# KamikaziZen/admm-quantization

Measured on AMD Instinct MI355X. Metric: ADMM iters/sec, resnet18 all conv layers 4-bit r=2.0; rel-Frob err vs CPU ref, higher is better.
Workload: dtype f32

## Files before the change

### admm-quantization_amd/admmq/_lib.py

```python
from __future__ import annotations

import ctypes
import os
from typing import Sequence

import torch

_HERE = os.path.dirname(os.path.abspath(__file__))
LIB_PATH = os.environ.get("ADMMQ_LIB") or os.path.join(_HERE, "libadmmq.so")

SCHEMES = {
    "tensor_mseminmax_symmetric": 0,
    "tensor_minmax": 1,
    "tensor_symmetric": 2,
    "tensor_affine": 3,
}
CHANNEL_SCHEMES = {"channel_symmetric": 4, "channel_affine": 5}


class AdmmProblem(ctypes.Structure):
    _fields_ = [("F", ctypes.c_void_p), ("G", ctypes.c_void_p), ("H0", ctypes.c_void_p),
                ("H_out", ctypes.c_void_p), ("U", ctypes.c_void_p), ("HT_out", ctypes.c_void_p),
                ("X_out", ctypes.c_void_p), ("I", ctypes.c_int32), ("R", ctypes.c_int32)]

# ... 41 lines not shown
def use_ops() -> bool:
    return not os.environ.get("ADMMQ_LIB")


def ops():
    global _ops
    if _ops is None:
        if not os.path.exists(OPS_PATH):
            raise ImportError(f"admmq: {OPS_PATH} is missing - build it with `make -C admm-quantization_amd/csrc`")
        load()
        torch.ops.load_library(OPS_PATH)
        _ops = torch.ops.admmq
    return _ops


def load() -> ctypes.CDLL:
    global _lib
    if _lib is not None:
        return _lib
    if not os.path.exists(LIB_PATH):
        raise ImportError(f"admmq: {LIB_PATH} is missing - build it with `python -c 'import __graft_entry__ as g; g.build()'` "
                          "or `make -C admm-quantization_amd/csrc`; there is no CPU fallback")
    lib = ctypes.CDLL(LIB_PATH)
    P, S, I32, I64, F32 = ctypes.c_void_p, ctypes.c_size_t, ctypes.c_int32, ctypes.c_int64, ctypes.c_float
    sig = {
        "admmq_admm_workspace_size": (S, [P, I32, I32]),
        "admmq_admm_prepare": (I32, [P, I32, I32, P, S, P]),
        "admmq_admm_run": (I32, [P, I32, I32, F32, I32, I32, I32, P, S, P, P]),
        "admmq_admm_iteration_batched": (I32, [P, I32, I32, F32, I32, I32, I32, P, S, P, P]),
        "admmq_admm_default_options": (I32, [P]),
        "admmq_admm_workspace_size_ex": (S, [P, I32, I32, P]),
        "admmq_admm_prepare_ex": (I32, [P, I32, I32, P, P, S, P]),
        "admmq_admm_run_ex": (I32, [P, I32, I32, F32, I32, I32, I32, P, P, S, P, P]),
        "admmq_debug_set_fin_wait_polls": (I32, [ctypes.c_uint32]),
        "admmq_debug_set_f32_persistent": (I32, [I32, I32]),
        "admmq_debug_set_gemm_ks": (I32, [I32]),
        "admmq_debug_set_gemm_stage": (I32, [I32]),
        "admmq_debug_set_ksplit": (I32, [I32]),
        "admmq_debug_set_ksplit_form": (I32, [I32]),
        "admmq_debug_set_ksplit_balance": (I32, [I32, I32]),
        "admmq_debug_ksplit_balance_count": (ctypes.c_int64, [ctypes.c_void_p, I32]),
        "admmq_debug_ksplit_pieces": (I32, [I32, I32]),
        "admmq_debug_set_even_units": (I32, [I32]),
        "admmq_spd_solve64": (I32, [P, P, I64, I64, P, P, P]),
        "admmq_debug_epc_evals": (I32, [P, I32]),
        "admmq_debug_spd_trace": (I32, [P]),
        "admmq_debug_epc_trace": (I32, [P]),
        "admmq_epc_step64": (I32, [P, P, I64, I64, ctypes.c_double, ctypes.c_double, P, P, P, P, P]),
        "admmq_debug_hist_cu": (I32, [P, I32]),
        "admmq_debug_set_fin_capacity": (I32, [I32]),
        "admmq_debug_set_fin_nv3": (I32, [I32]),
        "admmq_debug_set_thin_loop": (I32, [I32]),
        "admmq_quantize_workspace_size": (S, [P, I32, I32]),
        "admmq_quantize_batched": (I32, [P, I32, I32, I32, I32, P, S, P]),
        "admmq_packed_bytes": (S, [I64, I32]),
        "admmq_quantize_packed_workspace_size": (S, [P, I32, I32]),
        "admmq_quantize_packed": (I32, [P, P, P, I32, I32, I32, I32, P, S, P]),
        "admmq_dequantize_packed": (I32, [P, P, P, P, I32, P]),
        "admmq_packed_gemm_workspace_size": (S, [I64, I64, I64, I32]),
        "admmq_packed_gemm": (I32, [P, P, I32, I64, I64, P, I32, I64, I32, P, P, P, S, P]),
        "admmq_packed_dwgemm_workspace_size": (S, [I64, I64, I64, I64, I32]),
        "admmq_packed_dwgemm": (I32, [P, P, I64, I64, P, I32, I64, I64, P, I32, I32, I32, I32, I32, I32, P, P, P, S, P]),
        "admmq_fixed_quantize": (I32, [P, P, I64, P, P]),
        "admmq_packed_gemm_act": (I32, [P, P, I32, I64, I64, P, I32, I64, I32, P, P, P, P, S, P]),
        "admmq_packed_dwgemm_act": (I32, [P, P, I64, I64, P, I32, I64, I64, P, I32, I32, I32, I32, I32, I32, P, P, P, P, P,
                                          S, P]),
        "admmq_act_encode": (I32, [P, P, I64, P, P, P]),
        "admmq_act_decode": (I32, [P, P, I64, P, P]),
        "admmq_packed_rowsums": (I32, [P, P, I32, I64, I64, P, P]),
        "admmq_packed_igemm_workspace_size": (S, [I64, I64, I64, I32]),
        "admmq_packed_igemm": (I32, [P, P, I32, I64, I64, P, P, P, I32, I64, I32, P, P, P, P, P, P, S, P]),
        "admmq_mse_sse_table": (I32, [P, I64, I64, I32, I32, P, P, S, P]),
        "admmq_quantize_channel_workspace_size": (S, [P, I32, I32]),
        "admmq_quantize_channel": (I32, [P, P, P, I32, I32, I32, I32, P, S, P]),
        "admmq_set_exhaustive_search": (I32, [I32]),
        "admmq_debug_set_sel_widen": (I32, [I32]),
        "admmq_debug_shared_stage2_count": (I64, [I32]),
        "admmq_debug_set_wide_min_tiles": (I32, [ctypes.c_int64]),
        "admmq_set_solve_mode": (I32, [I32]),
        "admmq_get_solve_mode": (I32, []),
        "admmq_debug_set_legacy_stage1": (I32, [I32]),
        "admmq_debug_set_launch_head": (I32, [I32]),
        "admmq_debug_get_launch_head_default": (I32, []),
        "admmq_debug_admm_plan_bytes": (S, [P, I32, I32, P]),
        "admmq_debug_admm_plan_digest": (I32, [P, I32, I32, I32, P, P]),
        "admmq_debug_admm_run_schedule": (I32, [P, I32, I32, I32, I32, I32, I32, I32, I32, I32, P]),
        "admmq_debug_check_thresholds": (I32, [ctypes.c_uint32, I32]),
        "admmq_debug_set_fused_finalize": (I32, [I32]),
        "admmq_debug_set_search_units_per_block": (I32, [I32]),
        "admmq_debug_check_cells": (I32, [I32, I32, ctypes.c_uint32, I32, P]),
        "admmq_profile_begin": (I32, [I32, I32]),
        "admmq_profile_end": (I32, [P, P]),
        "admmq_cp_workspace_size": (S, [P, I32, I32]),
        "admmq_cp_gram_mttkrp": (I32, [P, I32, I32, P, S, P]),
        "admmq_cp_rel_error": (I32, [P, I32, P, P, S, P]),
        "admmq_cp64_workspace_size": (S, [P, I32, I32]),
        "admmq_cp64_gram_mttkrp": (I32, [P, I32, I32, P, S, P]),
        "admmq_lowrank_workspace_size": (S, [I64]),
        "admmq_lowrank_reset": (I32, [P, S, P]),
        "admmq_lowrank_pre": (I32, [P, P, P, P, P, P, I64, F32, P, S, P]),
        "admmq_lowrank_post": (I32, [P, P, P, P, I64, F32, P, S, P]),
        "admmq_panel_workspace_size": (S, [I64, I64, I64]),
        "admmq_panel_xtq": (I32, [P, I64, I64, I64, P, I64, P, P, S, P]),
        "admmq_panel_xy": (I32, [P, I64, I64, I64, P, I64, P, P, S, P]),
        "admmq_panel_outer": (I32, [P, P, I64, I64, I64, P, I64, P]),
        "admmq_gram64_workspace_size": (S, [I64, I64, I64]),
        "admmq_gram64": (I32, [P, I64, P, I64, I64, I64, I64, P, P, S, P]),
        "admmq_epc_mu": (I32, [P, P, I64, ctypes.c_double, ctypes.c_double, P, P]),
        "admmq_cp_colnorm64": (I32, [P, I64, P, I64, I64, P, P, P]),
        "admmq_solve64_workspace_size": (S, [I64, I64]),
        "admmq_epc64_max_evals": (I32, []),
        "admmq_debug_s64_evals": (I32, [P, I32]),
        "admmq_spd_solve64_ws": (I32, [P, P, I64, I64, ctypes.c_double, P, P, P, S, P]),
        "admmq_epc_begin64": (I32, [P, P, I64, I64, ctypes.c_double, ctypes.c_double, P, P, P, S, P]),
        "admmq_epc_rounds64": (I32, [P, P, I64, I64, P, I32, P, P, S, P]),
        "admmq_epc_end64": (I32, [I64, I64, P, P, P, S, P]),
        "admmq_version": (I32, []),
        "admmq_last_error": (ctypes.c_char_p, []),
    }
    for name, (res, args) in sig.items():
        if os.environ.get("ADMMQ_LIB") and not hasattr(lib, name):
            continue
        fn = getattr(lib, name)
        fn.restype = res
        fn.argtypes = args
    _lib = lib
    return lib


def check(rc: int, what: str):
    if rc != 0:
        msg = load().admmq_last_error().decode(errors="replace")
        raise RuntimeError(f"admmq: {what} failed (status {rc}): {msg}")


def require_device(*tensors: torch.Tensor):
    for t in tensors:
        if not isinstance(t, torch.Tensor):
            raise TypeError(f"admmq: expected a torch.Tensor, got {type(t).__name__}")
        if t.device.type != "cuda":
            raise RuntimeError("admmq: tensors must live on a ROCm GPU (device 'cuda'); the MI355X path has "
                               "no CPU implementation")
        if t.dtype != torch.float32:
            raise TypeError(f"admmq: float32 tensors required, got {t.dtype}")


def stream_handle(device: torch.device) -> ctypes.c_void_p:
    return ctypes.c_void_p(torch.cuda.current_stream(device).cuda_stream)


def ptr(t) -> ctypes.c_void_p:
    return ctypes.c_void_p(0 if t is None else t.data_ptr())


def workspace(nbytes: int, device: torch.device) -> torch.Tensor:
    return torch.empty(max(int(nbytes), 256), dtype=torch.uint8, device=device)


def problems_array(items: Sequence[AdmmProblem]):
    arr = (AdmmProblem * len(items))(*items)
    return arr


def qtensor_array(items: Sequence[QTensor]):
    return (QTensor * len(items))(*items)


_PY_REPAIRS = [0]


def note_repair(n: int = 1):
    _PY_REPAIRS[0] += n


def fault_repairs(reset: bool = False) -> int:
    n = _PY_REPAIRS[0]
    if reset:
        _PY_REPAIRS[0] = 0
    if use_ops():
        n += int(ops().fault_repairs(bool(reset)))
    return n


class _switch:

    _setter = ""
    _restore = 0
    _checked = (False, False)

    def _encode(self) -> int:
        return 1 if self.enable else 0

    def _set(self, value: int, checked: bool):
        rc = getattr(load(), self._setter)(value)
        if checked:
            check(rc, type(self).__name__)

    def __enter__(self):
        self._set(self._encode(), self._checked[0])
        return self

    def __exit__(self, *exc):
        self._set(self._restore, self._checked[1])
        return False


class exhaustive_search(_switch):

    _setter = "admmq_set_exhaustive_search"

    def __init__(self, enable: bool = True):
        self.enable = enable


class sel_widen(_switch):

    _setter, _checked = "admmq_debug_set_sel_widen", (True, True)

    def __init__(self, mode: int = 1):
        if mode not in (1, 2):
            raise ValueError(mode)
        self.mode = mode

    def _encode(self):
        return self.mode


def shared_stage2_count(reset: bool = False) -> int:
    n = int(load().admmq_debug_shared_stage2_count(1 if reset else 0))
    if n < 0:
        raise RuntimeError("admmq: shared_stage2_count failed")
    return n


class solve_mode:

    MODES = SOLVE_MODES

    def __init__(self, mode: str):
        if mode not in self.MODES:
            raise ValueError(mode)
        self.mode = mode

    def __enter__(self):
        self.prev = load().admmq_get_solve_mode()
        check(load().admmq_set_solve_mode(self.MODES[self.mode]), "set_solve_mode")
        return self

    def __exit__(self, *exc):
        load().admmq_set_solve_mode(self.prev)
        return False


class fin_nv3(_switch):

    _setter, _restore = "admmq_debug_set_fin_nv3", 1

    def __init__(self, enable: bool):
        self.enable = enable


class fused_finalize(_switch):

    _setter, _restore = "admmq_debug_set_fused_finalize", 1

    def __init__(self, enable: bool):
        self.enable = enable


class fin_wait_polls(_switch):

    _setter, _checked = "admmq_debug_set_fin_wait_polls", (True, False)

    def __init__(self, polls: int):
        self.polls = polls

    def _encode(self):
        return int(self.polls)


class fin_capacity(_switch):

    _setter, _checked = "admmq_debug_set_fin_capacity", (True, False)

    def __init__(self, blocks: int):
        self.blocks = blocks

    def _encode(self):
        return int(self.blocks)


class thin_loop(_switch):

    _setter, _restore, _checked = "admmq_debug_set_thin_loop", 1, (True, False)

    def __init__(self, enable):
        self.enable = enable

    def _encode(self):
        return 2 if self.enable == "wide" else (1 if self.enable else 0)


class search_units_per_block(_switch):

    _setter, _checked = "admmq_debug_set_search_units_per_block", (True, False)

    def __init__(self, reps: int):
        self.reps = reps

    def _encode(self):
# ... 15 lines not shown
```

### admm-quantization_amd/csrc/admmq_internal.h

```cpp
#pragma once
#include <hip/hip_runtime.h>
#include <stdint.h>

struct admmq_qmeta;

#ifndef ADMMQ_TRACE
#define ADMMQ_TRACE 0
#endif
#define ADMMQ_NOW() (ADMMQ_TRACE ? __builtin_amdgcn_s_memrealtime() : 0ull)

namespace admmq {

enum QScheme { kMse = 0, kMinMax = 1, kSymmetric = 2, kAffine = 3 };
enum SolveMode { kSolveF32 = 0, kSolveSplit = 1 };

constexpr int kMaxSel = 64;
constexpr int kMaxStage1 = 1024;
constexpr int kMaxStage1Bits = 6;
constexpr int kHistRep = 8;
constexpr int kMaxMerged = 4096;
constexpr int kCells = 4096;
constexpr int kResRep = 8;
constexpr int kThinRows = 16;
constexpr long long kWideMinTiles = 4 * 768;
constexpr int kWideRows = 256;

struct MseView {
  const float* X;
  const float* U;
  int rows, cols, ld, qpr;
  int nq, nelem;
  unsigned* stat;
  unsigned long long* sse;
  unsigned long long* h1;
  unsigned long long* h2;
  double* s2;
  int* sel;
  unsigned* ticket;
  unsigned long long* ready;
  const int* done;
  int nhist, pad_;
};

struct ProbDesc {
  const float* F_user;
  const float* G_user;
  const float* H0_user;
  float* H_out;
  float* U_user;
  float* HT_dbg;
  float* X_dbg;
  float* Fp; float* H; float* U; float* P; float* X; float* HT;
  float* M;
  double* A64; double* L64; double* D64;
  _Float16* P2; int* eP;
  _Float16* M2; int* eM;
  MseView mv;
  double* res;
  int* flags;
  float* rho;
  int I, R, ld, Ip, ldm, nbk;
  int nq;
  int split;
  int fin_rows;
  int ksplit;
  float* kpart;
  unsigned* kctr;
};

struct QJob {
  const float* src;
  float* dst;
  float* Xp;
  MseView mv;
  int rows, cols, ld, nq;
  float tmin_kw, tmax_kw;
  int has_kw, copy;
  unsigned* pstat;
  int pu0, pun;
};

constexpr int kDqJobs = 32;
constexpr int kDqBlockElems = 4096;
struct DqBatch {
  const unsigned char* codes[kDqJobs];
  float* y[kDqJobs];
  long long numel[kDqJobs];
  int blk0[kDqJobs + 1];
  int njobs, meta0;
};

struct GemmTile {
  int prob, tm, tn, nk;
  int ld, ldm;
  signed char first;
  unsigned char bm;
  short k0;
  signed char np, pc, ser, pad_;
  const float* P; const float* M; const float* U;
  const int* eP; const int* eM;
  float* part; unsigned* ctr;
  const int* flags; const double* res;
};
static_assert(sizeof(GemmTile) == 104, "GemmTile: the workspace carve depends on its size");
constexpr int kHeadGemmStop = 1;
constexpr int kLaunchHeadAll = kHeadGemmStop;
constexpr int kLaunchHeadDefault = kLaunchHeadAll;
constexpr int kKsplitMax = 4;
constexpr int kKsplitMinSteps = 6;
struct ThinLoopUnit { int job, col0, cw, rank, nteam, pad_[3]; };
constexpr int kTLThreads = 512;
constexpr int kTLMaxCand = 256;
constexpr int kTLBins = 264;
constexpr int kTLMaxTeam = 64;
constexpr int kTLKPairs = 9;
struct alignas(128) ThinSync {
  unsigned bar;
  unsigned pad0_[31];
  unsigned long long mx[2];
  unsigned long long pad1_[14];
  unsigned long long arr1[kTLMaxTeam];
  double s2[2];
  double res[2][4];
  double pad2_[6];
  unsigned long long h1[2][kTLBins];
  unsigned long long h2[2][kTLBins];
  unsigned long long sse[2][kTLBins];
};
struct Chunk {
  int job, start;
  const unsigned* stat;
  const int* done;
  const float* X;
  const float* U;
  long long total;
  const float* H;
  const float* F;
  const int* sel;
  int reps, step, nblk, pad2_;
};

typedef __attribute__((address_space(1))) const float gcf32;
typedef __attribute__((address_space(1))) const int gci32;
typedef float gf32x4 __attribute__((ext_vector_type(4)));
__device__ __forceinline__ float4 gld4(const float* q) {
  const gf32x4 v = *(__attribute__((address_space(1))) const gf32x4*)q;
  return make_float4(v.x, v.y, v.z, v.w);
}
__device__ __forceinline__ int gld_i32(const int* q) { return *(gci32*)q; }
__device__ __forceinline__ unsigned gld_u32(const unsigned* q) {
  return *(__attribute__((address_space(1))) const unsigned*)q;
}
__device__ __forceinline__ float4 sub4(float4 a, float4 b) {
  return make_float4(a.x - b.x, a.y - b.y, a.z - b.z, a.w - b.w);
}

__device__ __forceinline__ float4 load_x4(const float* X, const float* U, long long off) {
  float4 x = *reinterpret_cast<const float4*>(X + off);
  if (U) {
    const float4 u = *reinterpret_cast<const float4*>(U + off);
    x.x -= u.x; x.y -= u.y; x.z -= u.z; x.w -= u.w;
  }
  return x;
}

__device__ __forceinline__ unsigned enc_ord(float f) {
  unsigned b = __float_as_uint(f);
  return (b & 0x80000000u) ? ~b : (b | 0x80000000u);
}
__device__ __forceinline__ float dec_ord(unsigned e) {
  return __uint_as_float((e & 0x80000000u) ? (e & 0x7FFFFFFFu) : ~e);
}

int set_error(int code, const char* msg);
int upload_async(void* dst, const void* src, size_t n, hipStream_t s);

void launch_rho(const ProbDesc* d, int nprob, hipStream_t s);
void launch_pack(const ProbDesc* d, int nprob, int maxIp, int maxld, hipStream_t s);
void launch_fill_a64(const ProbDesc* d, int nprob, int maxldm, hipStream_t s);
void launch_spd_inverse(const ProbDesc* d, int nprob, int maxnbk, hipStream_t s);
void launch_spd_linv(const ProbDesc* d, int nprob, int maxnbk, hipStream_t s);
void launch_thin_solve(const ProbDesc* d, const ThinLoopUnit* units, int nunits, int nr, int maxld, int slot, int iter,
                       float eps, int ncand, hipStream_t s);
void launch_gemm(const ProbDesc* d, const GemmTile* tiles, int ntiles_wide, int ntiles_small, int ntiles_big,
                 bool split, int slot, int iter, float eps, int ncand, hipStream_t s, hipEvent_t ev0 = nullptr,
                 hipEvent_t ev1 = nullptr, bool prefetch_u = false);
extern int g_gemm_ks_f32;
int set_sel_widen_search(int on);
int set_sel_widen_thin(int on);
extern int g_gemm_f32_stage;
// ... 65 lines not shown
```

### admm-quantization_amd/csrc/spd_kernels.hip

```cpp
#include "admmq_internal.h"

namespace admmq {

constexpr int NB = 32;
constexpr int LS = NB + 1;

__device__ __forceinline__ void load_regs(double r[4], const double* A, int ldm, int bi, int bj);
__device__ __forceinline__ void store_regs(double* dst, const double r[4]);
__device__ __forceinline__ void load_block(double* dst, const double* A, int ldm, int bi, int bj) {
  double r[4];
  load_regs(r, A, ldm, bi, bj);
  store_regs(dst, r);
}
__device__ __forceinline__ void store_block(double* A, int ldm, int bi, int bj, const double* src) {
  for (int t = threadIdx.x; t < NB * NB; t += blockDim.x) {
    const int r = t >> 5, c = t & 31;
    A[(size_t)(bi * NB + r) * ldm + bj * NB + c] = src[r * LS + c];
  }
}

__device__ __forceinline__ void load_regs(double r[4], const double* A, int ldm, int bi, int bj) {
#pragma unroll
  for (int q = 0; q < 4; ++q) {
    const int t = threadIdx.x + 256 * q;
    r[q] = A[(size_t)(bi * NB + (t >> 5)) * ldm + bj * NB + (t & 31)];
  }
}
__device__ __forceinline__ void store_regs(double* dst, const double r[4]) {
#pragma unroll
  for (int q = 0; q < 4; ++q) {
    const int t = threadIdx.x + 256 * q;
    dst[(t >> 5) * LS + (t & 31)] = r[q];
  }
}

__device__ __forceinline__ double readlane_d(double v, int lane) {
  const long long b = __double_as_longlong(v);
  const int lo = __builtin_amdgcn_readlane((int)b, lane);
  const int hi = __builtin_amdgcn_readlane((int)(b >> 32), lane);
  return __longlong_as_double(((long long)hi << 32) | (unsigned)lo);
}

__device__ __forceinline__ double shfl_d(double v, int lane) {
  const long long b = __double_as_longlong(v);
  const int lo = __shfl((int)b, lane, 64);
  const int hi = __shfl((int)(b >> 32), lane, 64);
  return __longlong_as_double(((long long)hi << 32) | (unsigned)lo);
}

__device__ void chol32(double* a, int* err) {
  if (threadIdx.x < 64) {
    const int r = threadIdx.x & 31, h = threadIdx.x >> 5;
    double rw[NB / 2];
#pragma unroll
    for (int j = 0; j < NB / 2; ++j) rw[j] = a[r * LS + 2 * j + h];
#pragma unroll
    for (int c = 0; c < NB; ++c) {
      const double rc = shfl_d(rw[c >> 1], r + 32 * (c & 1));
      const double d = readlane_d(rw[c >> 1], c + 32 * (c & 1));
      if (threadIdx.x == 0 && !(d > 0.0)) *err = 1;
      const double sd = sqrt(d);
      const double l = r > c ? rc / sd : (r == c ? sd : 0.0);
      if ((c & 1) == h) rw[c >> 1] = l;
#pragma unroll
      for (int j = 0; j < NB / 2; ++j) {
        if (2 * j + 1 <= c) continue;
        const int sc = 2 * j + h;
        const double ls = shfl_d(l, sc);
        if (sc > c) rw[j] -= l * ls;
      }
    }
#pragma unroll
    for (int j = 0; j < NB / 2; ++j) {
      const int sc = 2 * j + h;
      a[r * LS + sc] = sc <= r ? rw[j] : 0.0;
    }
  }
  __syncthreads();
}

__device__ __forceinline__ void trinv32(const double* l, double* x) {
  if (threadIdx.x < NB) {
    const int c = threadIdx.x;
    x[c * LS + NB] = 1.0 / l[c * LS + c];
    __builtin_amdgcn_wave_barrier();
    asm volatile("" ::: "memory");
    double rinv[NB], col[NB];
#pragma unroll
    for (int r = 0; r < NB; ++r) rinv[r] = x[r * LS + NB];
#pragma unroll
    for (int r = 0; r < NB; ++r) {
      double lr[NB];
#pragma unroll
      for (int t = 0; t < r; ++t) lr[t] = l[r * LS + t];
      double s0 = 0.0, s1 = 0.0;
#pragma unroll
      for (int t = 0; t + 1 < r; t += 2) {
        s0 += lr[t] * col[t];
        s1 += lr[t + 1] * col[t + 1];
      }
      if (r & 1) s0 += lr[r - 1] * col[r - 1];
      col[r] = r < c ? 0.0 : (r == c ? rinv[r] : -(s0 + s1) * rinv[r]);
    }
#pragma unroll
    for (int r = 0; r < NB; ++r) x[r * LS + c] = col[r];
  }
  __syncthreads();
}

__device__ __forceinline__ void mm_nt(const double* a, const double* b, double acc[4]) {
  const int r = threadIdx.x >> 3, cb = (threadIdx.x & 7) * 4;
  for (int t = 0; t < NB; ++t) {
    const double av = a[r * LS + t];
#pragma unroll
    for (int q = 0; q < 4; ++q) acc[q] += av * b[(cb + q) * LS + t];
  }
}
__device__ __forceinline__ void mm_nn(const double* a, const double* b, double acc[4]) {
  const int r = threadIdx.x >> 3, cb = (threadIdx.x & 7) * 4;
  for (int t = 0; t < NB; ++t) {
    const double av = a[r * LS + t];
#pragma unroll
    for (int q = 0; q < 4; ++q) acc[q] += av * b[t * LS + cb + q];
  }
}
__device__ __forceinline__ void mm_tn(const double* a, const double* b, double acc[4]) {
  const int r = threadIdx.x >> 3, cb = (threadIdx.x & 7) * 4;
  for (int t = 0; t < NB; ++t) {
    const double av = a[t * LS + r];
#pragma unroll
    for (int q = 0; q < 4; ++q) acc[q] += av * b[t * LS + cb + q];
  }
}

__global__ __launch_bounds__(256) void k_chol_panel(const ProbDesc* __restrict__ probs, int k) {
  const ProbDesc& p = probs[blockIdx.y];
  const int i = k + blockIdx.x;
  if (k >= p.nbk || i >= p.nbk) return;
  __shared__ double lkk[NB * LS], x[NB * LS], aik[NB * LS];
  __shared__ int err;
  if (threadIdx.x == 0) err = 0;
  double ra[4];
  if (i != k) load_regs(ra, p.A64, p.ldm, i, k);
  load_block(lkk, p.A64, p.ldm, k, k);
  __syncthreads();
  chol32(lkk, &err);
  if (i == k) {
    if (err && threadIdx.x == 0) p.flags[2] = 1;
    store_block(p.D64, NB, k, 0, lkk);
    return;
  }
  trinv32(lkk, x);
  store_regs(aik, ra);
  __syncthreads();
  double acc[4] = {0.0, 0.0, 0.0, 0.0};
  mm_nt(aik, x, acc);
  __syncthreads();
  const int r = threadIdx.x >> 3, cb = (threadIdx.x & 7) * 4;
#pragma unroll
  for (int q = 0; q < 4; ++q) aik[r * LS + cb + q] = acc[q];
  __syncthreads();
  store_block(p.A64, p.ldm, i, k, aik);
}

__global__ __launch_bounds__(256) void k_chol_update(const ProbDesc* __restrict__ probs, int k) {
  const ProbDesc& p = probs[blockIdx.y];
  const int n = p.nbk - k - 1;
  if (n <= 0) return;
  const int q = blockIdx.x;
  if (q >= n * (n + 1) / 2) return;
  int ii = (int)((sqrt(8.0 * q + 1.0) - 1.0) * 0.5);
  while ((ii + 1) * (ii + 2) / 2 <= q) ++ii;
  while (ii * (ii + 1) / 2 > q) --ii;
  const int jj = q - ii * (ii + 1) / 2;
  const int i = k + 1 + ii, j = k + 1 + jj;
  __shared__ double li[NB * LS], lj[NB * LS];
  load_block(li, p.A64, p.ldm, i, k);
  load_block(lj, p.A64, p.ldm, j, k);
  __syncthreads();
  double acc[4] = {0.0, 0.0, 0.0, 0.0};
  mm_nt(li, lj, acc);
  const int r = threadIdx.x >> 3, cb = (threadIdx.x & 7) * 4;
  double* dst = p.A64 + (size_t)(i * NB + r) * p.ldm + j * NB + cb;
#pragma unroll
  for (int t = 0; t < 4; ++t) dst[t] -= acc[t];
}

__global__ __launch_bounds__(256) void k_linv_row(const ProbDesc* __restrict__ probs, int i) {
  const ProbDesc& p = probs[blockIdx.y];
  const int j = blockIdx.x;
  if (i >= p.nbk || j > i) return;
  __shared__ double lii[NB * LS], xi[NB * LS], ta[NB * LS], tb[NB * LS];
  load_block(lii, p.D64, NB, i, 0);
  __syncthreads();
  trinv32(lii, xi);
  if (j == i) {
    store_block(p.L64, p.ldm, i, i, xi);
    return;
  }
  double acc[4] = {0.0, 0.0, 0.0, 0.0};
  double ra[4], rb[4];
  if (j < i) { load_regs(ra, p.A64, p.ldm, i, j); load_regs(rb, p.L64, p.ldm, j, j); }
  for (int t = j; t < i; ++t) {
    store_regs(ta, ra);
    store_regs(tb, rb);
    __syncthreads();
    if (t + 1 < i) { load_regs(ra, p.A64, p.ldm, i, t + 1); load_regs(rb, p.L64, p.ldm, t + 1, j); }
    mm_nn(ta, tb, acc);
    __syncthreads();
  }
  const int r = threadIdx.x >> 3, cb = (threadIdx.x & 7) * 4;
#pragma unroll
  for (int q = 0; q < 4; ++q) ta[r * LS + cb + q] = acc[q];
  __syncthreads();
  double out[4] = {0.0, 0.0, 0.0, 0.0};
  mm_nn(xi, ta, out);
  __syncthreads();
#pragma unroll
  for (int q = 0; q < 4; ++q) tb[r * LS + cb + q] = -out[q];
  __syncthreads();
  store_block(p.L64, p.ldm, i, j, tb);
}

__global__ __launch_bounds__(256) void k_diag_inv(const ProbDesc* __restrict__ probs) {
  const ProbDesc& p = probs[blockIdx.y];
  const int i = blockIdx.x;
  if (i >= p.nbk) return;
  __shared__ double lii[NB * LS], xi[NB * LS];
  load_block(lii, p.D64, NB, i, 0);
  __syncthreads();
  trinv32(lii, xi);
  store_block(p.L64, p.ldm, i, i, xi);
}

constexpr int kLinvCols = 4;
constexpr int kLinvGroups = 8;
constexpr int kLinvMaxNbk = 56;
constexpr int kLinvPer = (kLinvMaxNbk + kLinvGroups - 1) / kLinvGroups;
__global__ __launch_bounds__(1024) void k_linv_cols(const ProbDesc* __restrict__ probs) {
  const ProbDesc& p = probs[blockIdx.y];
  constexpr int nsl = NB / kLinvCols;
  const int j = blockIdx.x / nsl, c0 = (blockIdx.x % nsl) * kLinvCols;
  const int nbk = p.nbk, ldm = p.ldm;
  if (j >= nbk - 1) return;
  extern __shared__ double linv_lds[];
  double* panel = linv_lds;
  double* sbuf = linv_lds + (size_t)(gridDim.x / nsl + 1) * NB * kLinvCols;
  const int g = threadIdx.x >> 7, lt = threadIdx.x & 127;
  const int r = lt >> 2, c = lt & 3;
  const double* A64 = p.A64;
  double* L64 = p.L64;
  if (g == 0)
    panel[(j * NB + r) * kLinvCols + c] = L64[(size_t)(j * NB + r) * ldm + j * NB + c0 + c];
  double acc[kLinvPer];
#pragma unroll
  for (int q = 0; q < kLinvPer; ++q) acc[q] = 0.0;
  __syncthreads();
  for (int t = j; t < nbk - 1; ++t) {
    const double* pt = panel + t * NB * kLinvCols + c;
#pragma unroll
    for (int q = 0; q < kLinvPer; ++q) {
      const int i = j + 1 + g + kLinvGroups * q;
      if (i > t && i < nbk) {
        const double2* lp = reinterpret_cast<const double2*>(A64 + (size_t)(i * NB + r) * ldm + t * NB);
        double a = acc[q];
#pragma unroll
        for (int k = 0; k < NB; k += 2) {
          const double2 x = lp[k / 2];
          a += x.x * pt[k * kLinvCols];
          a += x.y * pt[(k + 1) * kLinvCols];
        }
        acc[q] = a;
      }
    }
    const int i = t + 1;
    const int og = (i - j - 1) % kLinvGroups, oq = (i - j - 1) / kLinvGroups;
    if (g == og) {
      double v = 0.0;
#pragma unroll
      for (int q = 0; q < kLinvPer; ++q) v = q == oq ? acc[q] : v;
      sbuf[r * kLinvCols + c] = v;
    }
    __syncthreads();
    if (g == og) {
      const double2* dp = reinterpret_cast<const double2*>(L64 + (size_t)(i * NB + r) * ldm + i * NB);
      double o = 0.0;
#pragma unroll
      for (int k = 0; k < NB; k += 2) {
        const double2 d = dp[k / 2];
        o += d.x * sbuf[k * kLinvCols + c];
        o += d.y * sbuf[(k + 1) * kLinvCols + c];
      }
      panel[(i * NB + r) * kLinvCols + c] = -o;
      L64[(size_t)(i * NB + r) * ldm + j * NB + c0 + c] = -o;
    }
    __syncthreads();
  }
}

__global__ __launch_bounds__(256) void k_minv(const ProbDesc* __restrict__ probs) {
  const ProbDesc& p = probs[blockIdx.y];
  const int q = blockIdx.x;
  const int n = p.nbk;
  if (q >= n * (n + 1) / 2) return;
  int i = (int)((sqrt(8.0 * q + 1.0) - 1.0) * 0.5);
  while ((i + 1) * (i + 2) / 2 <= q) ++i;
  while (i * (i + 1) / 2 > q) --i;
  const int j = q - i * (i + 1) / 2;
  __shared__ double ta[NB * LS], tb[NB * LS];
  double acc[4] = {0.0, 0.0, 0.0, 0.0};
  double ra[4], rb[4];
  load_regs(ra, p.L64, p.ldm, i, i);
  load_regs(rb, p.L64, p.ldm, i, j);
  for (int t = i; t < n; ++t) {
    store_regs(ta, ra);
    store_regs(tb, rb);
    __syncthreads();
    if (t + 1 < n) { load_regs(ra, p.L64, p.ldm, t + 1, i); load_regs(rb, p.L64, p.ldm, t + 1, j); }
    mm_tn(ta, tb, acc);
    __syncthreads();
  }
  const int r = threadIdx.x >> 3, cb = (threadIdx.x & 7) * 4;
  const int gr = i * NB + r;
#pragma unroll
  for (int t = 0; t < 4; ++t) {
    const int gc = j * NB + cb + t;
    const float v = (gr < p.R && gc < p.R) ? (float)acc[t] : 0.f;
    p.M[(size_t)gr * p.ldm + gc] = v;
    p.M[(size_t)gc * p.ldm + gr] = v;
  }
}

void launch_spd_linv(const ProbDesc* d, int nprob, int maxnbk, hipStream_t s) {
  for (int k = 0; k < maxnbk; ++k) {
    hipLaunchKernelGGL(k_chol_panel, dim3(maxnbk - k, nprob), dim3(256), 0, s, d, k);
    const int n = maxnbk - k - 1;
    if (n > 0) hipLaunchKernelGGL(k_chol_update, dim3(n * (n + 1) / 2, nprob), dim3(256), 0, s, d, k);
  }
  if (maxnbk <= kLinvMaxNbk) {
    hipLaunchKernelGGL(k_diag_inv, dim3(maxnbk, nprob), dim3(256), 0, s, d);
    if (maxnbk > 1)
      hipLaunchKernelGGL(k_linv_cols, dim3((maxnbk - 1) * (NB / kLinvCols), nprob), dim3(1024),
                         (size_t)(maxnbk + 1) * NB * kLinvCols * sizeof(double), s, d);
  } else {
    for (int i = 0; i < maxnbk; ++i) hipLaunchKernelGGL(k_linv_row, dim3(i + 1, nprob), dim3(256), 0, s, d, i);
  }
}

void launch_spd_inverse(const ProbDesc* d, int nprob, int maxnbk, hipStream_t s) {
  launch_spd_linv(d, nprob, maxnbk, s);
  hipLaunchKernelGGL(k_minv, dim3(maxnbk * (maxnbk + 1) / 2, nprob), dim3(256), 0, s, d);
}

}
```

Measured before the change: 270,700.

## Fuse Cholesky panel and trailing update into one step kernel; widen L-inverse and M-inverse tiles

Replaces the two per-step launches of the blocked Cholesky (panel, then trailing update) with a single flattened k_chol_step launch. In each step the trailing update lagged from the previous step is applied inside the panel work, which halves the number of kernel launches and dependency boundaries. It also adds a templated column-sliced L-inverse kernel that uses narrower column slices (width 4 by default for small block counts) to spread the work over more blocks. The last change is an M-inverse kernel in which 128 threads each compute a 2x4 register tile. All three paths are on by default and selected through a form mask; the price is more complex indexing and a lagged-update order that must keep the results numerically equivalent.

```diff
diff --git a/admm-quantization_amd/admmq/_lib.py b/admm-quantization_amd/admmq/_lib.py
--- a/admm-quantization_amd/admmq/_lib.py
+++ b/admm-quantization_amd/admmq/_lib.py
@@ -147,6 +147,12 @@
         "admmq_debug_set_legacy_stage1": (I32, [I32]),
         "admmq_debug_set_launch_head": (I32, [I32]),
         "admmq_debug_get_launch_head_default": (I32, []),
+        "admmq_debug_set_spd_form": (I32, [I32]),
+        "admmq_debug_get_spd_form_default": (I32, []),
+        "admmq_debug_set_linv_width": (I32, [I32]),
+        "admmq_debug_linv_width": (I32, [I32]),
+        "admmq_debug_chol_step_work": (I32, [I32, I32, P, I32, P]),
+        "admmq_debug_spd_inverse": (I32, [I32, P, P, ctypes.c_double, P, P, P, P, P, I32, P]),
         "admmq_debug_admm_plan_bytes": (S, [P, I32, I32, P]),
         "admmq_debug_admm_plan_digest": (I32, [P, I32, I32, I32, P, P]),
         "admmq_debug_admm_run_schedule": (I32, [P, I32, I32, I32, I32, I32, I32, I32, I32, I32, P]),
@@ -291,6 +297,61 @@
         return self.mode
 
 
+SPD_FUSED_CHOL, SPD_WIDE_LINV, SPD_TILE_MINV = 1, 2, 4
+
+
+class spd_form:
+
+    def __init__(self, mask=None, linv_width: int = 0):
+        self.default = load().admmq_debug_get_spd_form_default()
+        self.mask = self.default if mask is None else mask
+        self.width = linv_width
+
+    def __enter__(self):
+        check(load().admmq_debug_set_spd_form(self.mask), "spd_form")
+        check(load().admmq_debug_set_linv_width(self.width), "linv_width")
+        return self
+
+    def __exit__(self, *exc):
+        check(load().admmq_debug_set_spd_form(self.default), "spd_form")
+        check(load().admmq_debug_set_linv_width(0), "linv_width")
+        return False
+
+
+def chol_step_work(s: int, nbk: Sequence[int]):
+    arr = (ctypes.c_int32 * len(nbk))(*nbk)
+    out = (ctypes.c_int32 * 3)()
+    n = load().admmq_debug_chol_step_work(s, len(nbk), arr, 0, out)
+    if n < 0:
+        raise ValueError("chol_step_work: bad arguments")
+    work = []
+    for wid in range(n):
+        if load().admmq_debug_chol_step_work(s, len(nbk), arr, wid, out) != n:
+            raise RuntimeError("chol_step_work failed")
+        if out[0] >= 0:
+            work.append((int(out[0]), int(out[1]), int(out[2])))
+    return work, n
+
+
+def debug_spd_inverse(Gs, shift: float = 0.0, reps: int = 1):
+    import numpy as np
+    n = len(Gs)
+    Gs = [np.ascontiguousarray(g, dtype=np.float64) for g in Gs]
+    R = [g.shape[0] for g in Gs]
+    ldm = [(r + 31) // 32 * 32 for r in R]
+    out = [dict(M=np.empty((l, l), np.float32), A=np.empty((l, l), np.float64), Linv=np.empty((l, l), np.float64),
+                D=np.empty((l, 32), np.float64)) for l in ldm]
+    vp = lambda arrs: (ctypes.c_void_p * n)(*[a.ctypes.data for a in arrs])
+    flags = (ctypes.c_int32 * n)()
+    ms = ctypes.c_float(0.0)
+    check(load().admmq_debug_spd_inverse(n, (ctypes.c_int32 * n)(*R), vp(Gs), float(shift), vp([o["M"] for o in out]),
+                                         vp([o["A"] for o in out]), vp([o["Linv"] for o in out]),
+                                         vp([o["D"] for o in out]), flags, reps, ctypes.byref(ms)), "debug_spd_inverse")
+    for o, f in zip(out, flags):
+        o["flag"] = int(f)
+    return out, float(ms.value)
+
+
 def shared_stage2_count(reset: bool = False) -> int:
     n = int(load().admmq_debug_shared_stage2_count(1 if reset else 0))
     if n < 0:
diff --git a/admm-quantization_amd/csrc/admmq_internal.h b/admm-quantization_amd/csrc/admmq_internal.h
--- a/admm-quantization_amd/csrc/admmq_internal.h
+++ b/admm-quantization_amd/csrc/admmq_internal.h
@@ -106,6 +106,11 @@
 constexpr int kHeadGemmStop = 1;
 constexpr int kLaunchHeadAll = kHeadGemmStop;
 constexpr int kLaunchHeadDefault = kLaunchHeadAll;
+constexpr int kSpdFusedChol = 1;
+constexpr int kSpdWideLinv = 2;
+constexpr int kSpdTileMinv = 4;
+constexpr int kSpdFormAll = kSpdFusedChol | kSpdWideLinv | kSpdTileMinv;
+constexpr int kSpdFormDefault = kSpdFormAll;
 constexpr int kKsplitMax = 4;
 constexpr int kKsplitMinSteps = 6;
 struct ThinLoopUnit { int job, col0, cw, rank, nteam, pad_[3]; };
diff --git a/admm-quantization_amd/csrc/spd_kernels.hip b/admm-quantization_amd/csrc/spd_kernels.hip
--- a/admm-quantization_amd/csrc/spd_kernels.hip
+++ b/admm-quantization_amd/csrc/spd_kernels.hip
@@ -1,3 +1,9 @@
+#include <algorithm>
+#include <atomic>
+#include <cstring>
+#include <vector>
+
+#include "../../include/admmq.h"
 #include "admmq_internal.h"
 
 namespace admmq {
@@ -48,8 +54,8 @@
   return __longlong_as_double(((long long)hi << 32) | (unsigned)lo);
 }
 
-__device__ void chol32(double* a, int* err) {
-  if (threadIdx.x < 64) {
+__device__ __forceinline__ void chol32_wave(double* a, int* err) {
+  {
     const int r = threadIdx.x & 31, h = threadIdx.x >> 5;
     double rw[NB / 2];
 #pragma unroll
@@ -76,11 +82,14 @@
       a[r * LS + sc] = sc <= r ? rw[j] : 0.0;
     }
   }
-  __syncthreads();
-}
-
-__device__ __forceinline__ void trinv32(const double* l, double* x) {
-  if (threadIdx.x < NB) {
+}
+__device__ void chol32(double* a, int* err) {
+  if (threadIdx.x < 64) chol32_wave(a, err);
+  __syncthreads();
+}
+
+__device__ __forceinline__ void trinv32_cols(const double* l, double* x) {
+  {
     const int c = threadIdx.x;
     x[c * LS + NB] = 1.0 / l[c * LS + c];
     __builtin_amdgcn_wave_barrier();
@@ -105,16 +114,21 @@
 #pragma unroll
     for (int r = 0; r < NB; ++r) x[r * LS + c] = col[r];
   }
-  __syncthreads();
-}
-
-__device__ __forceinline__ void mm_nt(const double* a, const double* b, double acc[4]) {
-  const int r = threadIdx.x >> 3, cb = (threadIdx.x & 7) * 4;
+}
+__device__ __forceinline__ void trinv32(const double* l, double* x) {
+  if (threadIdx.x < NB) trinv32_cols(l, x);
+  __syncthreads();
+}
+
+__device__ __forceinline__ void mm_nt_at(const double* a, const double* b, double acc[4], int r, int cb) {
   for (int t = 0; t < NB; ++t) {
     const double av = a[r * LS + t];
 #pragma unroll
     for (int q = 0; q < 4; ++q) acc[q] += av * b[(cb + q) * LS + t];
   }
+}
+__device__ __forceinline__ void mm_nt(const double* a, const double* b, double acc[4]) {
+  mm_nt_at(a, b, acc, threadIdx.x >> 3, (threadIdx.x & 7) * 4);
 }
 __device__ __forceinline__ void mm_nn(const double* a, const double* b, double acc[4]) {
   const int r = threadIdx.x >> 3, cb = (threadIdx.x & 7) * 4;
@@ -184,6 +198,124 @@
   double* dst = p.A64 + (size_t)(i * NB + r) * p.ldm + j * NB + cb;
 #pragma unroll
   for (int t = 0; t < 4; ++t) dst[t] -= acc[t];
+}
+
+struct CholStepWork { int prob, i, j; };
+__host__ __device__ inline int chol_step_cols(int s, int maxnbk) { return maxnbk - s; }
+__host__ __device__ inline int chol_step_trail(int s, int maxnbk) {
+  const int n = maxnbk - s - 1;
+  return s > 0 ? n * (n + 1) / 2 : 0;
+}
+__host__ __device__ inline CholStepWork chol_step_work(int s, int maxnbk, int nprob, int id) {
+  const int ncol = chol_step_cols(s, maxnbk);
+  CholStepWork w;
+  if (id < ncol * nprob) {
+    w.prob = id / ncol;
+    w.i = s + id % ncol;
+    w.j = s;
+    return w;
+  }
+  const int e = id - ncol * nprob, ntr = chol_step_trail(s, maxnbk);
+  w.prob = e / ntr;
+  const int q = e % ntr;
+  int ii = (int)((sqrt(8.0 * q + 1.0) - 1.0) * 0.5);
+  while ((ii + 1) * (ii + 2) / 2 <= q) ++ii;
+  while (ii * (ii + 1) / 2 > q) --ii;
+  w.i = s + 1 + ii;
+  w.j = s + 1 + (q - ii * (ii + 1) / 2);
+  return w;
+}
+
+__global__ __launch_bounds__(256) void k_chol_step(const ProbDesc* __restrict__ probs, int s, int maxnbk, int nprob) {
+  const CholStepWork w = chol_step_work(s, maxnbk, nprob, blockIdx.x);
+  const ProbDesc& p = probs[w.prob];
+  const int i = w.i, j = w.j, ldm = p.ldm;
+  if (i >= p.nbk) return;
+  __shared__ double b0[NB * LS], b1[NB * LS], b2[NB * LS];
+  __shared__ int err;
+  const int r = threadIdx.x >> 3, cb = (threadIdx.x & 7) * 4;
+  if (j > s) {
+    load_block(b0, p.A64, ldm, i, s - 1);
+    load_block(b1, p.A64, ldm, j, s - 1);
+    __syncthreads();
+    double acc[4] = {0.0, 0.0, 0.0, 0.0};
+    mm_nt(b0, b1, acc);
+    double* dst = p.A64 + (size_t)(i * NB + r) * ldm + j * NB + cb;
+#pragma unroll
+    for (int t = 0; t < 4; ++t) dst[t] -= acc[t];
+    return;
+  }
+  if (threadIdx.x == 0) err = 0;
+  double rs[4], rp[4], rl[4];
+  load_regs(rs, p.A64, ldm, s, s);
+  if (s > 0) {
+    load_regs(rp, p.A64, ldm, s, s - 1);
+    if (i != s) load_regs(rl, p.A64, ldm, i, s - 1);
+  }
+  double v[2][4];
+  if (i != s && threadIdx.x >= 64) {
+#pragma unroll
+    for (int m = 0; m < 2; ++m) {
+      const int st = threadIdx.x - 64 + 192 * m;
+      if (st < 256) {
+        const double* src = p.A64 + (size_t)(i * NB + (st >> 3)) * ldm + s * NB + (st & 7) * 4;
+#pragma unroll
+        for (int q = 0; q < 4; ++q) v[m][q] = src[q];
+      }
+    }
+  }
+  store_regs(b0, rs);
+  if (s > 0) {
+    store_regs(b1, rp);
+    if (i != s) store_regs(b2, rl);
+  }
+  __syncthreads();
+  if (s > 0) {
+    double acc[4] = {0.0, 0.0, 0.0, 0.0};
+    mm_nt(b1, b1, acc);
+#pragma unroll
+    for (int q = 0; q < 4; ++q) b0[r * LS + cb + q] -= acc[q];
+    __syncthreads();
+  }
+  if (threadIdx.x < 64) {
+    chol32_wave(b0, &err);
+  } else if (i != s && s > 0) {
+#pragma unroll
+    for (int m = 0; m < 2; ++m) {
+      const int st = threadIdx.x - 64 + 192 * m;
+      if (st < 256) {
+        double acc[4] = {0.0, 0.0, 0.0, 0.0};
+        mm_nt_at(b2, b1, acc, st >> 3, (st & 7) * 4);
+#pragma unroll
+        for (int q = 0; q < 4; ++q) v[m][q] -= acc[q];
+      }
+    }
+  }
+  __syncthreads();
+  if (i == s) {
+    if (err && threadIdx.x == 0) p.flags[2] = 1;
+    store_block(p.D64, NB, s, 0, b0);
+    return;
+  }
+  if (threadIdx.x < NB) {
+    trinv32_cols(b0, b1);
+  } else if (threadIdx.x >= 64) {
+#pragma unroll
+    for (int m = 0; m < 2; ++m) {
+      const int st = threadIdx.x - 64 + 192 * m;
+      if (st < 256) {
+#pragma unroll
+        for (int q = 0; q < 4; ++q) b2[(st >> 3) * LS + (st & 7) * 4 + q] = v[m][q];
+      }
+    }
+  }
+  __syncthreads();
+  double acc[4] = {0.0, 0.0, 0.0, 0.0};
+  mm_nt(b2, b1, acc);
+#pragma unroll
+  for (int q = 0; q < 4; ++q) b0[r * LS + cb + q] = acc[q];
+  __syncthreads();
+  store_block(p.A64, ldm, i, s, b0);
 }
 
 __global__ __launch_bounds__(256) void k_linv_row(const ProbDesc* __restrict__ probs, int i) {
@@ -295,6 +427,142 @@
       L64[(size_t)(i * NB + r) * ldm + j * NB + c0 + c] = -o;
     }
     __syncthreads();
+  }
+}
+
+constexpr int kLinvMaxNbk16 = 38;
+constexpr int kLinvWideThreads = 64 * kLinvGroups;
+constexpr int kLinvMidNbk = 40;
+template <int W, int CAP>
+__global__ __launch_bounds__(kLinvWideThreads, W == 4 ? 4 : 2) void k_linv_cols_w(const ProbDesc* __restrict__ probs) {
+  constexpr int nsl = NB / W, kCpt = W / 2, kPer = (CAP + kLinvGroups - 1) / kLinvGroups;
+  const ProbDesc& p = probs[blockIdx.y];
+  const int j = blockIdx.x / nsl, c0 = (blockIdx.x % nsl) * W;
+  const int nbk = p.nbk, ldm = p.ldm;
+  if (j >= nbk - 1) return;
+  extern __shared__ double linv_lds[];
+  double* panel = linv_lds;
+  double* sbuf = linv_lds + (size_t)(gridDim.x / nsl + 1) * NB * W;
+  const int g = threadIdx.x >> 6, lt = threadIdx.x & 63;
+  const int r = lt >> 1, c = (lt & 1) * kCpt;
+  const double* A64 = p.A64;
+  double* L64 = p.L64;
+  if (g == 0) {
+#pragma unroll
+    for (int m = 0; m < kCpt; ++m)
+      panel[(j * NB + r) * W + c + m] = L64[(size_t)(j * NB + r) * ldm + j * NB + c0 + c + m];
+  }
+  double acc[kPer][kCpt];
+#pragma unroll
+  for (int q = 0; q < kPer; ++q)
+#pragma unroll
+    for (int m = 0; m < kCpt; ++m) acc[q][m] = 0.0;
+  __syncthreads();
+  for (int t = j; t < nbk - 1; ++t) {
+    const double* pt = panel + t * NB * W + c;
+#pragma unroll
+    for (int q = 0; q < kPer; ++q) {
+      const int i = j + 1 + g + kLinvGroups * q;
+      if (i > t && i < nbk) {
+        const double2* lp = reinterpret_cast<const double2*>(A64 + (size_t)(i * NB + r) * ldm + t * NB);
+#pragma unroll
+        for (int h = 0; h < 2; ++h) {
+          double2 x[NB / 4];
+#pragma unroll
+          for (int k = 0; k < NB / 4; ++k) x[k] = lp[h * (NB / 4) + k];
+#pragma unroll
+          for (int k = 0; k < NB / 2; k += 2) {
+#pragma unroll
+            for (int m = 0; m < kCpt; ++m) acc[q][m] += x[k / 2].x * pt[(h * (NB / 2) + k) * W + m];
+#pragma unroll
+            for (int m = 0; m < kCpt; ++m) acc[q][m] += x[k / 2].y * pt[(h * (NB / 2) + k + 1) * W + m];
+          }
+        }
+      }
+    }
+    const int i = t + 1;
+    const int og = (i - j - 1) % kLinvGroups, oq = (i - j - 1) / kLinvGroups;
+    double2 d[NB / 2];
+    const double2* dp = reinterpret_cast<const double2*>(L64 + (size_t)(i * NB + r) * ldm + i * NB);
+    if (g == og) {
+#pragma unroll
+      for (int k = 0; k < NB / 4; ++k) d[k] = dp[k];
+#pragma unroll
+      for (int m = 0; m < kCpt; ++m) {
+        double v = 0.0;
+#pragma unroll
+        for (int q = 0; q < kPer; ++q) v = q == oq ? acc[q][m] : v;
+        sbuf[r * W + c + m] = v;
+      }
+    }
+    __syncthreads();
+    if (g == og) {
+#pragma unroll
+      for (int k = NB / 4; k < NB / 2; ++k) d[k] = dp[k];
+      double o[kCpt];
+#pragma unroll
+      for (int m = 0; m < kCpt; ++m) o[m] = 0.0;
+#pragma unroll
+      for (int k = 0; k < NB; k += 2) {
+#pragma unroll
+        for (int m = 0; m < kCpt; ++m) o[m] += d[k / 2].x * sbuf[k * W + c + m];
+#pragma unroll
+        for (int m = 0; m < kCpt; ++m) o[m] += d[k / 2].y * sbuf[(k + 1) * W + c + m];
+      }
+#pragma unroll
+      for (int m = 0; m < kCpt; ++m) {
+        panel[(i * NB + r) * W + c + m] = -o[m];
+        L64[(size_t)(i * NB + r) * ldm + j * NB + c0 + c + m] = -o[m];
+      }
+    }
+    __syncthreads();
+  }
+}
+
+__global__ __launch_bounds__(256) void k_minv_tile(const ProbDesc* __restrict__ probs) {
+  const ProbDesc& p = probs[blockIdx.y];
+  const int q = blockIdx.x;
+  const int n = p.nbk;
+  if (q >= n * (n + 1) / 2) return;
+  int i = (int)((sqrt(8.0 * q + 1.0) - 1.0) * 0.5);
+  while ((i + 1) * (i + 2) / 2 <= q) ++i;
+  while (i * (i + 1) / 2 > q) --i;
+  const int j = q - i * (i + 1) / 2;
+  __shared__ double ta[NB * LS], tb[NB * LS];
+  const int r0 = ((threadIdx.x >> 3) & 15) * 2, cb = (threadIdx.x & 7) * 4;
+  double acc[2][4] = {{0.0, 0.0, 0.0, 0.0}, {0.0, 0.0, 0.0, 0.0}};
+  double ra[4], rb[4];
+  load_regs(ra, p.L64, p.ldm, i, i);
+  load_regs(rb, p.L64, p.ldm, i, j);
+  for (int t = i; t < n; ++t) {
+    store_regs(ta, ra);
+    store_regs(tb, rb);
+    __syncthreads();
+    if (t + 1 < n) { load_regs(ra, p.L64, p.ldm, t + 1, i); load_regs(rb, p.L64, p.ldm, t + 1, j); }
+    if (threadIdx.x < 128) {
+      for (int k = 0; k < NB; ++k) {
+        const double a0 = ta[k * LS + r0], a1 = ta[k * LS + r0 + 1];
+#pragma unroll
+        for (int m = 0; m < 4; ++m) {
+          const double bv = tb[k * LS + cb + m];
+          acc[0][m] += a0 * bv;
+          acc[1][m] += a1 * bv;
+        }
+      }
+    }
+    __syncthreads();
+  }
+  if (threadIdx.x >= 128) return;
+#pragma unroll
+  for (int h = 0; h < 2; ++h) {
+    const int gr = i * NB + r0 + h;
+#pragma unroll
+    for (int t = 0; t < 4; ++t) {
+      const int gc = j * NB + cb + t;
+      const float v = (gr < p.R && gc < p.R) ? (float)acc[h][t] : 0.f;
+      p.M[(size_t)gr * p.ldm + gc] = v;
+      p.M[(size_t)gc * p.ldm + gr] = v;
+    }
   }
 }
 
@@ -331,17 +599,50 @@
   }
 }
 
+static std::atomic<int> g_spd_form{kSpdFormDefault};
+static std::atomic<int> g_linv_width{0};
+
+static int linv_width(int maxnbk) {
+  if (!(g_spd_form.load() & kSpdWideLinv)) return kLinvCols;
+  const int w = g_linv_width.load();
+  if (w == 16 && maxnbk <= kLinvMaxNbk16) return 16;
+  if (w == 8 || w == 16) return 8;
+  return maxnbk <= kLinvMidNbk ? 2 : kLinvCols;
+}
+
+template <int W, int CAP>
+static void launch_linv_cols_w(const ProbDesc* d, int nprob, int maxnbk, hipStream_t s) {
+  const size_t lds = (size_t)(maxnbk + 1) * NB * W * sizeof(double);
+  if (lds > 64 * 1024)
+    (void)hipFuncSetAttribute(reinterpret_cast<const void*>(k_linv_cols_w<W, CAP>), hipFuncAttributeMaxDynamicSharedMemorySize,
+                              (int)lds);
+  hipLaunchKernelGGL((k_linv_cols_w<W, CAP>), dim3((maxnbk - 1) * (NB / W), nprob), dim3(kLinvWideThreads), lds, s, d);
+}
+
 void launch_spd_linv(const ProbDesc* d, int nprob, int maxnbk, hipStream_t s) {
-  for (int k = 0; k < maxnbk; ++k) {
-    hipLaunchKernelGGL(k_chol_panel, dim3(maxnbk - k, nprob), dim3(256), 0, s, d, k);
-    const int n = maxnbk - k - 1;
-    if (n > 0) hipLaunchKernelGGL(k_chol_update, dim3(n * (n + 1) / 2, nprob), dim3(256), 0, s, d, k);
+  if (g_spd_form.load() & kSpdFusedChol) {
+    for (int k = 0; k < maxnbk; ++k) {
+      const int nwg = nprob * (chol_step_cols(k, maxnbk) + chol_step_trail(k, maxnbk));
+      hipLaunchKernelGGL(k_chol_step, dim3(nwg), dim3(256), 0, s, d, k, maxnbk, nprob);
+    }
+  } else {
+    for (int k = 0; k < maxnbk; ++k) {
+      hipLaunchKernelGGL(k_chol_panel, dim3(maxnbk - k, nprob), dim3(256), 0, s, d, k);
+      const int n = maxnbk - k - 1;
+      if (n > 0) hipLaunchKernelGGL(k_chol_update, dim3(n * (n + 1) / 2, nprob), dim3(256), 0, s, d, k);
+    }
   }
   if (maxnbk <= kLinvMaxNbk) {
     hipLaunchKernelGGL(k_diag_inv, dim3(maxnbk, nprob), dim3(256), 0, s, d);
-    if (maxnbk > 1)
-      hipLaunchKernelGGL(k_linv_cols, dim3((maxnbk - 1) * (NB / kLinvCols), nprob), dim3(1024),
-                         (size_t)(maxnbk + 1) * NB * kLinvCols * sizeof(double), s, d);
+    if (maxnbk > 1) {
+      const int w = linv_width(maxnbk);
+      if (w == 16) launch_linv_cols_w<16, kLinvMaxNbk16>(d, nprob, maxnbk, s);
+      else if (w == 8) launch_linv_cols_w<8, kLinvMaxNbk>(d, nprob, maxnbk, s);
+      else if (w == 2) launch_linv_cols_w<4, kLinvMidNbk>(d, nprob, maxnbk, s);
+      else
+        hipLaunchKernelGGL(k_linv_cols, dim3((maxnbk - 1) * (NB / kLinvCols), nprob), dim3(1024),
+                           (size_t)(maxnbk + 1) * NB * kLinvCols * sizeof(double), s, d);
+    }
   } else {
     for (int i = 0; i < maxnbk; ++i) hipLaunchKernelGGL(k_linv_row, dim3(i + 1, nprob), dim3(256), 0, s, d, i);
   }
@@ -349,7 +650,128 @@
 
 void launch_spd_inverse(const ProbDesc* d, int nprob, int maxnbk, hipStream_t s) {
   launch_spd_linv(d, nprob, maxnbk, s);
-  hipLaunchKernelGGL(k_minv, dim3(maxnbk * (maxnbk + 1) / 2, nprob), dim3(256), 0, s, d);
-}
-
-}
+  const dim3 grid(maxnbk * (maxnbk + 1) / 2, nprob);
+  if (g_spd_form.load() & kSpdTileMinv) hipLaunchKernelGGL(k_minv_tile, grid, dim3(256), 0, s, d);
+  else hipLaunchKernelGGL(k_minv, grid, dim3(256), 0, s, d);
+}
+
+__global__ __launch_bounds__(256) void k_spd_debug_fill(const ProbDesc* __restrict__ probs, const double* const* __restrict__ G,
+                                                        double shift) {
+  const ProbDesc& p = probs[blockIdx.y];
+  const double* g = G[blockIdx.y];
+  const long long total = (long long)p.ldm * p.ldm;
+  for (long long e = (long long)blockIdx.x * 256 + threadIdx.x; e < total; e += (long long)gridDim.x * 256) {
+    const int r = (int)(e / p.ldm), c = (int)(e - (long long)r * p.ldm);
+    double v;
+    if (r < p.R && c < p.R) v = g[(size_t)r * p.R + c] + (r == c ? shift : 0.0);
+    else v = r == c ? 1.0 : 0.0;
+    p.A64[e] = v;
+  }
+}
+
+}
+
+using namespace admmq;
+
+extern "C" {
+
+int32_t admmq_debug_set_spd_form(int32_t mask) {
+  if (mask < 0 || (mask & ~kSpdFormAll)) return set_error(ADMMQ_ERR_ARG, "spd form mask out of range");
+  g_spd_form = mask;
+  return ADMMQ_OK;
+}
+int32_t admmq_debug_get_spd_form_default(void) { return kSpdFormDefault; }
+int32_t admmq_debug_set_linv_width(int32_t w) {
+  if (w != 0 && w != 8 && w != 16) return set_error(ADMMQ_ERR_ARG, "linv width must be 0, 8 or 16");
+  g_linv_width = w;
+  return ADMMQ_OK;
+}
+int32_t admmq_debug_linv_width(int32_t maxnbk) { return maxnbk >= 2 && maxnbk <= kLinvMaxNbk ? linv_width(maxnbk) : 0; }
+
+int32_t admmq_debug_chol_step_work(int32_t s, int32_t nprob, const int32_t* nbk, int32_t id, int32_t* out) {
+  if (!nbk || !out || nprob < 1 || s < 0) return -1;
+  int maxnbk = 0;
+  for (int q = 0; q < nprob; ++q) maxnbk = std::max(maxnbk, nbk[q]);
+  if (s >= maxnbk) return -1;
+  const int nwg = nprob * (chol_step_cols(s, maxnbk) + chol_step_trail(s, maxnbk));
+  if (id < 0 || id >= nwg) return -1;
+  const CholStepWork w = chol_step_work(s, maxnbk, nprob, id);
+  const bool on = w.i < nbk[w.prob];
+  out[0] = on ? w.prob : -1; out[1] = w.i; out[2] = w.j;
+  return nwg;
+}
+
+int32_t admmq_debug_spd_inverse(int32_t nprob, const int32_t* R, const double* const* G, double shift, float* const* M,
+                                double* const* A, double* const* Linv, double* const* D, int32_t* flags2, int32_t reps,
+                                float* ms) {
+  if (nprob < 1 || nprob > 64 || !R || !G || reps < 1) return set_error(ADMMQ_ERR_ARG, "spd_inverse: bad arguments");
+  std::vector<ProbDesc> desc(nprob);
+  std::vector<const double*> dG(nprob);
+  std::vector<void*> owned;
+  auto dev = [&](size_t bytes) -> void* {
+    void* q = nullptr;
+    if (hipMalloc(&q, bytes) != hipSuccess) return nullptr;
+    owned.push_back(q);
+    return q;
+  };
+  auto done = [&](int rc, const char* msg) {
+    (void)hipDeviceSynchronize();
+    for (void* q : owned) (void)hipFree(q);
+    return rc == ADMMQ_OK ? rc : set_error(rc, msg);
+  };
+  int maxnbk = 0, maxldm = 0;
+  int* dflags = static_cast<int*>(dev((size_t)nprob * 4 * sizeof(int)));
+  if (!dflags || hipMemset(dflags, 0, (size_t)nprob * 4 * sizeof(int)) != hipSuccess) return done(ADMMQ_ERR_HIP, "spd_inverse: alloc");
+  for (int q = 0; q < nprob; ++q) {
+    if (R[q] < 1 || R[q] > 8192 || !G[q]) return done(ADMMQ_ERR_ARG, "spd_inverse: bad problem");
+    ProbDesc& d = desc[q];
+    std::memset(&d, 0, sizeof(d));
+    d.R = R[q]; d.ldm = (R[q] + NB - 1) / NB * NB; d.nbk = d.ldm / NB;
+    const size_t l2 = (size_t)d.ldm * d.ldm;
+    d.A64 = static_cast<double*>(dev(l2 * 8));
+    d.L64 = static_cast<double*>(dev(l2 * 8));
+    d.D64 = static_cast<double*>(dev((size_t)d.ldm * NB * 8));
+    d.M = static_cast<float*>(dev(l2 * 4));
+    double* g = static_cast<double*>(dev((size_t)R[q] * R[q] * 8));
+    d.flags = dflags + 4 * q;
+    if (!d.A64 || !d.L64 || !d.D64 || !d.M || !g) return done(ADMMQ_ERR_HIP, "spd_inverse: alloc");
+    if (hipMemset(d.L64, 0, l2 * 8) != hipSuccess || hipMemset(d.M, 0, l2 * 4) != hipSuccess ||
+        hipMemcpy(g, G[q], (size_t)R[q] * R[q] * 8, hipMemcpyHostToDevice) != hipSuccess)
+      return done(ADMMQ_ERR_HIP, "spd_inverse: upload");
+    dG[q] = g;
+    maxnbk = std::max(maxnbk, d.nbk);
+    maxldm = std::max(maxldm, d.ldm);
+  }
+  ProbDesc* ddesc = static_cast<ProbDesc*>(dev(nprob * sizeof(ProbDesc)));
+  const double** ddG = static_cast<const double**>(dev(nprob * sizeof(double*)));
+  hipEvent_t e0 = nullptr, e1 = nullptr;
+  if (!ddesc || !ddG || hipMemcpy(ddesc, desc.data(), nprob * sizeof(ProbDesc), hipMemcpyHostToDevice) != hipSuccess ||
+      hipMemcpy(ddG, dG.data(), nprob * sizeof(double*), hipMemcpyHostToDevice) != hipSuccess ||
+      hipEventCreate(&e0) != hipSuccess || hipEventCreate(&e1) != hipSuccess)
+    return done(ADMMQ_ERR_HIP, "spd_inverse: upload");
+  const int fb = (int)std::min<long long>(1024, ((long long)maxldm * maxldm + 255) / 256);
+  for (int it = 0; it < reps; ++it) {
+    hipLaunchKernelGGL(k_spd_debug_fill, dim3(fb, nprob), dim3(256), 0, nullptr, ddesc, ddG, shift);
+    (void)hipEventRecord(e0, nullptr);
+    launch_spd_inverse(ddesc, nprob, maxnbk, nullptr);
+    (void)hipEventRecord(e1, nullptr);
+  }
+  float t = 0.f;
+  bool ok = hipEventSynchronize(e1) == hipSuccess && hipEventElapsedTime(&t, e0, e1) == hipSuccess;
+  (void)hipEventDestroy(e0); (void)hipEventDestroy(e1);
+  if (ms) *ms = t;
+  std::vector<int> hf((size_t)nprob * 4);
+  ok = ok && hipMemcpy(hf.data(), dflags, hf.size() * sizeof(int), hipMemcpyDeviceToHost) == hipSuccess;
+  for (int q = 0; ok && q < nprob; ++q) {
+    const ProbDesc& d = desc[q];
+    const size_t l2 = (size_t)d.ldm * d.ldm;
+    if (flags2) flags2[q] = hf[4 * q + 2];
+    if (M && M[q]) ok = ok && hipMemcpy(M[q], d.M, l2 * 4, hipMemcpyDeviceToHost) == hipSuccess;
+    if (A && A[q]) ok = ok && hipMemcpy(A[q], d.A64, l2 * 8, hipMemcpyDeviceToHost) == hipSuccess;
+    if (Linv && Linv[q]) ok = ok && hipMemcpy(Linv[q], d.L64, l2 * 8, hipMemcpyDeviceToHost) == hipSuccess;
+    if (D && D[q]) ok = ok && hipMemcpy(D[q], d.D64, (size_t)d.ldm * NB * 8, hipMemcpyDeviceToHost) == hipSuccess;
+  }
+  return done(ok ? ADMMQ_OK : ADMMQ_ERR_HIP, "spd_inverse: run failed");
+}
+
+}
```

New measurement: 273,400, median of 6. 1.01x the previous value.
